# hila-chefer/Transformer-Explainability

Hardware: AMD Instinct MI355X
Metric: relevance maps/sec (ViT-B/16 224^2, batch 64 per GPU, generate_LRP transformer_attribution) (higher is better)
Workload: dtype f32 (3xbf16 split operands, 6 products, fp32 accumulate)

## Files before the change

include/te_relprop.h:

```cpp
#ifndef TE_RELPROP_H
#define TE_RELPROP_H

#include <stddef.h>
#include <stdint.h>

#ifdef __cplusplus
extern "C" {
#endif

typedef void* te_stream_t;
typedef uint16_t te_bf16_t;

enum {
  TE_OK = 0,
  TE_ERR_INVALID_ARG = -1,
  TE_ERR_WORKSPACE = -2,
  TE_ERR_UNSUPPORTED = -3,
  TE_ERR_NO_DEVICE = -4
};

enum { TE_VARIANT_OURS = 0, TE_VARIANT_LRP = 1, TE_IMPL_SIMPLE = 0x100 };

enum { TE_ROLLOUT_NORMALISE = 1, TE_ROLLOUT_CLS_FIXUP = 2, TE_ROLLOUT_ROW0 = 4 };

// ... 102 lines not shown
                                const float* R1, const float* s1, int64_t s1_stride,
                                const float* R2, const float* s2, int64_t s2_stride,
                                const float* X, float* out, int64_t B, int64_t n, te_stream_t stream);

int te_index_select_relprop_f32(const float* R, const float* X, float* out,
                                int64_t B, int64_t N, int64_t C, int64_t index, te_stream_t stream);

int te_gradcam_headmean_f32(const float* grad, const float* cam, float* out,
                            int64_t B, int64_t H, int64_t N, te_stream_t stream);

size_t te_rollout_workspace_bytes(int64_t L, int64_t B, int64_t N);
size_t te_rollout_row0_workspace_bytes(int64_t B, int64_t N);
int te_rollout_f32(const float* cams, int64_t L, int64_t start_layer, int64_t B, int64_t N,
                   int flags, float* joint, void* ws, size_t ws_bytes, te_stream_t stream);

#define TE_X6_TILE_AUTO 0
#define TE_X6_TILE_128 1
#define TE_X6_TILE_256 2
#define TE_X6_TILE_128x128 3
#define TE_X6_TEST_DROP_HANDOVER 0x200
#define TE_X6_WHOLE_TILES 0x10000
#define TE_X6_TEST_SMALL_GRID 0x4000
#define TE_X6_X_PLANES_SIGNED 0x20000
#define TE_X6_TILE_Z_SHIFT 10
#define TE_X6_TILE_C_SHIFT 12
#define TE_X6_PHASE_SPLIT 4
#define TE_X6_PHASE_Z 8
#define TE_X6_PHASE_C 16
#define TE_X6_PHASE_MASK 28
int te_linear_relprop_x6_supported(int64_t T, int64_t in_f, int64_t out_f);
size_t te_linear_relprop_x6_workspace_bytes(int64_t T, int64_t in_f, int64_t out_f);
size_t te_linear_x6_weight_planes_bytes(int64_t in_f, int64_t out_f);
size_t te_linear_x6_planes_bytes(int64_t rows, int64_t K);
int te_linear_x6_prepare_weights_f32(const float* W, int64_t in_f, int64_t out_f, void* planes, size_t planes_bytes,
                                     te_stream_t stream);
int te_linear_x6_split_abs_f32(const float* X, int64_t rows, int64_t K, void* planes, size_t planes_bytes,
                               te_stream_t stream);
int te_linear_relprop_x6_f32(const float* R, const float* r_scale, int64_t r_scale_stride, int64_t rows_per_sample,
                             const float* X, const float* W, const void* w_planes, const void* x_planes,
                             const float* Y, const float* bias, float* out,
                             int64_t T, int64_t in_f, int64_t out_f, int flags, unsigned* status, void* ws,
                             size_t ws_bytes, te_stream_t stream);
int te_linear_relprop_x6_check(const void* ws, int64_t T, int64_t in_f, int64_t out_f, te_stream_t stream);

int te_linear_relprop_x6_general_supported(int64_t T, int64_t in_f, int64_t out_f, int variant);
size_t te_linear_x6_weight_planes_lrp_bytes(int64_t in_f, int64_t out_f);
// ... 293 lines not shown
```

transformer-explainability_amd/csrc/te_api.hip:

```cpp
#include "te_common.h"

#include <string.h>

extern "C" int te_version(void) { return 706;  }

#ifndef TE_BUILD_ID
#define TE_BUILD_ID "unstamped"
#endif
extern "C" const char* te_build_id(void) { return TE_BUILD_ID; }

extern "C" const char* te_status_string(int status) {
  switch (status) {
    case TE_OK: return "ok";
    case TE_ERR_INVALID_ARG: return "invalid argument";
    case TE_ERR_WORKSPACE: return "workspace missing, misaligned or too small";
    case TE_ERR_UNSUPPORTED: return "shape not supported by the gfx950 kernels";
    case TE_ERR_NO_DEVICE: return "no gfx950 device visible";
    default: break;
  }
  if (status > 0) return hipGetErrorString((hipError_t)status);
  return "unknown status";
}

extern "C" int te_device_check(void) {
  int n = 0;
  if (hipGetDeviceCount(&n) != hipSuccess || n <= 0) return TE_ERR_NO_DEVICE;
  for (int d = 0; d < n; ++d) {
// ... 7 lines not shown
```

transformer-explainability_amd/csrc/te_linear_x6.hip:

```cpp
#include <algorithm>
#include <cmath>
#include <type_traits>

#include "te_x6.h"

namespace {

constexpr int kRB = 3 * kFrag;
constexpr int kMinFrag = 4;
constexpr float kCancelTol = 0.0078125f;
constexpr int kSpinMillis = 250;
constexpr int kErrWord = 1023;


enum { MODE_Z = 0, MODE_C = 1, MODE_G = 2, MODE_ZI = 3, MODE_Z1 = 4, MODE_CI = 5, MODE_X = 6, MODE_ZS = 7 };

__device__ __forceinline__ float bf16_f32(unsigned b) { return __uint_as_float(b << 16); }

enum { OP_ABS = 0, OP_POS = 1, OP_NEG = 2, OP_ID = 3 };
template <int OP>
__device__ __forceinline__ float apply_op(float x) {
  if constexpr (OP == OP_ID) return x;
  if constexpr (OP == OP_ABS) return __int_as_float(__float_as_int(x) & 0x7fffffff);
  const int b = __float_as_int(x);
  if constexpr (OP == OP_POS) return __int_as_float(b > 0 ? b : 0);
  return __int_as_float(b < 0 ? b : 0);
}

template <int OP, bool TRANSPOSE>
__global__ __launch_bounds__(256) void split_kernel(const float* __restrict__ src, unsigned char* __restrict__ dst,
                                                    int64_t R, int64_t K, int group, int sign,
                                                    unsigned char* __restrict__ dst_abs = nullptr) {
  const int r = threadIdx.x & 31, sl = threadIdx.x >> 5;
  const int64_t rb = blockIdx.x;
  const int64_t ks = (int64_t)blockIdx.y * 8 + sl;
  const int64_t nks = K >> 4;
  if (ks >= nks) return;
  const int64_t row = rb * 32 + r;
// ... 186 lines not shown
#else
#define X6_PASS4(a, b, c, d) (void)0
#endif

__device__ __forceinline__ void glds16(const unsigned char* src, unsigned char* lds_wave_base) {
  __builtin_amdgcn_global_load_lds((const __attribute__((address_space(1))) void*)src,
                                   (__attribute__((address_space(3))) void*)lds_wave_base, 16, 0, 0);
}

constexpr int kStages = 2;
template <int WM>
struct X6Geo {
  static constexpr int NWM = (WM == 1) ? 1 : 2, NWN = (WM == 0) ? 2 : 4, MI = (WM == 0) ? 2 : 4;
  static constexpr int NW = NWM * NWN, THREADS = 64 * NW, WPS = (WM == 0) ? 3 : 2;
  static constexpr int TM = NWM * MI * 32, TT = NWN * 64;
  static constexpr int NPA = 3 * NWM * MI, NPB = 3 * NWN * 2;
  static constexpr int ACC = MI * 2 * 16;
  static constexpr int MAX_SPX = (WM == 2) ? 32 : (WM == 1) ? 64 : 96;
};

template <int WM, int MODE>
struct X6Lds {
  using GEO = X6Geo<WM>;
  static constexpr bool STAGED = (MODE == MODE_Z || MODE == MODE_ZS || MODE == MODE_ZI || MODE == MODE_Z1) && GEO::MI == 4;
  static constexpr int STAGES = kStages * (GEO::NPA + GEO::NPB) * kFrag;
  static constexpr int MAIN = (STAGED && GEO::NW * 16384 > STAGES) ? GEO::NW * 16384 : STAGES;
  static constexpr int TOTAL = MAIN + GEO::NW * 512 + 16;
};

template <int WM, int MODE>
__global__ __launch_bounds__(X6Geo<WM>::THREADS, X6Geo<WM>::WPS) void x6_kernel(const X6Params p) {
  using GEO = X6Geo<WM>;
  constexpr int NW = GEO::NW, NWM = GEO::NWM, NWN = GEO::NWN, MI = GEO::MI;
  constexpr bool SGN = MODE == MODE_ZS;
  constexpr bool Z_ABS = MODE == MODE_Z || SGN;
  constexpr bool IS_Z = (Z_ABS || MODE == MODE_ZI || MODE == MODE_Z1);
  constexpr bool IS_C = (MODE == MODE_C || MODE == MODE_CI);
  constexpr int G = IS_C ? 6 : 3;
  constexpr int NPA = GEO::NPA, NPB = GEO::NPB;
  constexpr int NP = NPA + NPB;
  static_assert(NPA / 3 == NW, "each wave stages one weight-side block");
  constexpr int PBW = NPB / 3 / NW;
  constexpr int STAGE = NP * kFrag;
  constexpr int GROUPS = NPA / G;
  constexpr int LDS_MAIN = X6Lds<WM, MODE>::MAIN;
  extern __shared__ __attribute__((aligned(16))) unsigned char smem[];

  const int lane = threadIdx.x & 63;
  const int wave = __builtin_amdgcn_readfirstlane(threadIdx.x >> 6);
  const int wm = wave / NWN, wn = wave % NWN;
  const int lane16 = lane * 16;

  const int bid = blockIdx.x, spx = gridDim.x >> 3;
  const int xcd = bid & 7, slot = bid >> 3;
  const int nks = p.nks;
  const int tiles = p.ntm * p.ntn;
  const int tx0 = (int)((int64_t)tiles * xcd / 8), tx1 = (int)((int64_t)tiles * (xcd + 1) / 8);
  const int ntx = tx1 - tx0;
// ... 21 lines not shown
  for (int seq = 0; seq < nseq; ++seq) {
    int tile, k0, k1;
    if (head && seq == 0) {
      tile = l_tile, k0 = 0, k1 = ke;
    } else if (tail && seq == nseq - 1) {
      tile = f_tile, k0 = kb, k1 = (f_tile == l_tile) ? ke : nks;
    } else {
      tile = full0 + seq - (head ? 1 : 0), k0 = 0, k1 = nks;
    }
    tile += tx0;
    int tn, tm;
    if (p.t_fast) {
      tm = tile / p.ntn, tn = tile - tm * p.ntn;
    } else {
      tn = tile / p.ntm, tm = tile - tn * p.ntm;
    }

    const unsigned char* srcA;
    if constexpr (!IS_C)
      srcA = p.A + (int64_t)(tm * GROUPS + wave) * p.a_group_stride + (int64_t)k0 * kRB;
    else
      srcA = p.A + (int64_t)(tm * GROUPS + (wave >> 1)) * p.a_group_stride + (int64_t)k0 * (2 * kRB) + (wave & 1) * kRB;
    const unsigned char* srcB[PBW];
#pragma unroll
    for (int u = 0; u < PBW; ++u) {
      const int cb = min(tn * (GEO::TT / 32) + wave * PBW + u, p.ncb - 1);
      srcB[u] = p.B + (int64_t)cb * p.b_rb_stride + (int64_t)k0 * kRB;
    }
    unsigned char* const ldsA = smem + wave * kRB;
    unsigned char* const ldsB = smem + NPA * kFrag + wave * (PBW * kRB);
    u32x4 breg[SGN ? PBW : 1][3];
    auto stage_in = [&](int stg, int adv) __attribute__((always_inline)) {
      srcA += adv * (G * kFrag);
#pragma unroll
      for (int u = 0; u < PBW; ++u) srcB[u] += adv * kRB;
#pragma unroll
      for (int q = 0; q < 3; ++q) glds16(srcA + q * kFrag + lane16, ldsA + stg * STAGE + q * kFrag);
#pragma unroll
      for (int u = 0; u < PBW; ++u)
#pragma unroll
        for (int q = 0; q < 3; ++q) {
          if constexpr (SGN) breg[u][q] = *reinterpret_cast<const u32x4*>(srcB[u] + q * kFrag + lane16);
          else glds16(srcB[u] + q * kFrag + lane16, ldsB + stg * STAGE + (u * 3 + q) * kFrag);
        }
    };
    auto sign_and_store = [&](int stg) __attribute__((always_inline)) {
#pragma unroll
      for (int u = 0; u < (SGN ? PBW : 0); ++u) {
#pragma unroll
        for (int e = 0; e < 4; ++e) {
          const unsigned m = breg[u][0][e] & 0x80008000u;
          breg[u][0][e] &= 0x7fff7fffu;
          breg[u][1][e] ^= m;
          breg[u][2][e] ^= m;
        }
#pragma unroll
        for (int q = 0; q < 3; ++q) *reinterpret_cast<u32x4*>(ldsB + stg * STAGE + (u * 3 + q) * kFrag + lane16) = breg[u][q];
      }
    };

    auto wait_for = [&](unsigned* flag) -> bool {
      unsigned* const ok_word = reinterpret_cast<unsigned*>(smem + LDS_MAIN + NW * 512);
      if (threadIdx.x == 0) {
        unsigned spins = 0, ok = 1u;
        const long long t_begin = wall_clock64();
        while (__hip_atomic_load(flag, __ATOMIC_RELAXED, __HIP_MEMORY_SCOPE_AGENT) == 0u) {
          __builtin_amdgcn_s_sleep(8);
// ... 23 lines not shown
      for (int mi = 0; mi < MI; ++mi)
#pragma unroll
        for (int ni = 0; ni < 2; ++ni) {
#pragma unroll
          for (int c = 0; c < 4; ++c) {
            const f32x4 v = ip[c * 64];
#pragma unroll
            for (int e = 0; e < 4; ++e) acc[mi][ni][4 * c + e] = handed_over ? v[e] : __builtin_nanf("");
          }
          ip += 4 * 64;
          asm volatile("" : "+v"(ip));
        }
    } else {
#pragma unroll
      for (int mi = 0; mi < MI; ++mi)
#pragma unroll
        for (int ni = 0; ni < 2; ++ni)
#pragma unroll
          for (int e = 0; e < 16; ++e) acc[mi][ni][e] = 0.0f;
    }

    stage_in(0, 0);
    if constexpr (SGN) sign_and_store(0);
    int st = 0;
    bf16x8 a[MI][3], b[2][3];
    for (int ks = k0; ks < k1; ++ks) {
      asm volatile("s_waitcnt vmcnt(0) lgkmcnt(0)" ::: "memory");
      __builtin_amdgcn_s_barrier();
      const unsigned char* sA = smem + st * STAGE + wm * (MI * kRB) + lane16;
      const unsigned char* sB = smem + st * STAGE + NPA * kFrag + wn * (2 * kRB) + lane16;
      const unsigned aA = (unsigned)(uintptr_t)sA, aB = (unsigned)(uintptr_t)sB;
#define X6_SB __builtin_amdgcn_sched_barrier(0)
#define X6_RDB(ni, r) \
  asm volatile("ds_read_b128 %0, %1 offset:%2" : "=v"(b[ni][PB[r]]) : "v"(aB), "i"((ni) * kRB + PB[r] * kFrag))
#define X6_RDA(mi, r) \
  asm volatile("ds_read_b128 %0, %1 offset:%2" : "=v"(a[mi][PA[r]]) : "v"(aA), "i"((mi) * kRB + PA[r] * kFrag))
#define X6_WAIT(n)                                                           \
  X6_SB;                                                                     \
  asm volatile("s_waitcnt lgkmcnt(" #n ")" ::: "memory"); \
  X6_SB
#define X6_MM(mi, ni, q) acc[mi][ni] = TE_MFMA_BF16(a[mi][PA[q]], b[ni][PB[q]], acc[mi][ni])
#define X6_RD_HEAD(r) X6_SB; X6_RDB(0, r); X6_RDA(0, r); X6_RDA(1, r); X6_SB
#define X6_RD_TAIL(r) X6_SB; X6_RDB(1, r); X6_RDA(2, r); X6_RDA(3, r); X6_SB
      if constexpr (MI == 2) {
#define X6_RD4(r) X6_SB; X6_RDB(0, r); X6_RDA(0, r); X6_RDA(1, r); X6_RDB(1, r); X6_SB
        X6_RD4(0);
        X6_RD4(1);
        stage_in((st + 1) % kStages, (ks + 1 < k1) ? 1 : 0);
        X6_WAIT(6); X6_MM(0, 0, 0);
        X6_WAIT(5); X6_MM(1, 0, 0);
        X6_WAIT(4); X6_MM(1, 1, 0); X6_MM(0, 1, 0);
        X6_RD4(2);
        X6_WAIT(6); X6_MM(0, 0, 1);
        X6_WAIT(5); X6_MM(1, 0, 1);
        X6_WAIT(4); X6_MM(1, 1, 1); X6_MM(0, 1, 1);
        X6_WAIT(2); X6_MM(0, 0, 2);
        X6_WAIT(1); X6_MM(1, 0, 2);
        X6_WAIT(0); X6_MM(1, 1, 2); X6_MM(0, 1, 2);
        X6_SB;
#pragma unroll
        for (int q6 = 3; q6 < 6; ++q6) {
          X6_MM(0, 0, q6); X6_MM(1, 0, q6); X6_MM(1, 1, q6); X6_MM(0, 1, q6);
          X6_SB;
        }
#undef X6_RD4
      } else {
      X6_RD_HEAD(0);
      X6_RD_TAIL(0);
      stage_in((st + 1) % kStages, (ks + 1 < k1) ? 1 : 0);
      X6_WAIT(4); X6_MM(0, 0, 0);
      X6_WAIT(3); X6_MM(1, 0, 0);
      X6_WAIT(2); X6_MM(1, 1, 0); X6_MM(0, 1, 0);
      X6_RD_HEAD(1);
      X6_WAIT(4); X6_MM(2, 1, 0); X6_MM(2, 0, 0);
      X6_WAIT(3); X6_MM(3, 0, 0); X6_MM(3, 1, 0);
      X6_RD_TAIL(1);
      X6_WAIT(4); X6_MM(0, 0, 1);
      X6_WAIT(3); X6_MM(1, 0, 1);
      X6_WAIT(2); X6_MM(1, 1, 1); X6_MM(0, 1, 1);
      X6_RD_HEAD(2);
      X6_WAIT(4); X6_MM(2, 1, 1); X6_MM(2, 0, 1);
      X6_WAIT(3); X6_MM(3, 0, 1); X6_MM(3, 1, 1);
      X6_RD_TAIL(2);
      X6_WAIT(4); X6_MM(0, 0, 2);
      X6_WAIT(3); X6_MM(1, 0, 2);
      X6_WAIT(2); X6_MM(1, 1, 2); X6_MM(0, 1, 2);
      X6_WAIT(1); X6_MM(2, 1, 2); X6_MM(2, 0, 2);
      X6_WAIT(0); X6_MM(3, 0, 2); X6_MM(3, 1, 2);
      X6_SB;
#pragma unroll
      for (int q6 = 3; q6 < 6; ++q6) {
        X6_MM(0, 0, q6); X6_MM(1, 0, q6); X6_MM(1, 1, q6); X6_MM(0, 1, q6);
        X6_MM(2, 1, q6); X6_MM(2, 0, q6); X6_MM(3, 0, q6); X6_MM(3, 1, q6);
        X6_SB;
      }
      }
#undef X6_SB
#undef X6_RDB
#undef X6_RDA
#undef X6_WAIT
#undef X6_MM
#undef X6_RD_HEAD
#undef X6_RD_TAIL
      if constexpr (SGN) sign_and_store((st + 1) % kStages);
      st = (st + 1 == kStages) ? 0 : st + 1;
    }
    if constexpr (SGN) asm volatile("s_waitcnt lgkmcnt(0)" ::: "memory");

    auto publish = [&](float* dst, unsigned* flag) __attribute__((always_inline)) {
      f32x4* op = reinterpret_cast<f32x4*>(dst) + (size_t)wave * (GEO::ACC / 4) * 64 + lane;
#pragma unroll
      for (int mi = 0; mi < MI; ++mi)
#pragma unroll
        for (int ni = 0; ni < 2; ++ni) {
#pragma unroll
          for (int c = 0; c < 4; ++c) {
            f32x4 v;
#pragma unroll
            for (int e = 0; e < 4; ++e) v[e] = acc[mi][ni][4 * c + e];
            op[c * 64] = v;
          }
          op += 4 * 64;
          asm volatile("" : "+v"(op));
        }
      asm volatile("s_waitcnt vmcnt(0)" ::: "memory");
      __syncthreads();
      if (threadIdx.x == 0) {
        __builtin_amdgcn_fence(__ATOMIC_RELEASE, "agent");
        asm volatile("s_waitcnt vmcnt(0)" ::: "memory");
        if (!p.drop_handover) __hip_atomic_store(flag, 1u, __ATOMIC_RELAXED, __HIP_MEMORY_SCOPE_AGENT);
// ... 249 lines not shown
          if (__builtin_amdgcn_ballot_w64(bad != 0) != 0) {
            asm volatile("s_waitcnt vmcnt(0)" ::: "memory");
            const float* Rrow = p.R + tl[ni] * p.out_f;
#pragma clang loop unroll(disable)
            for (int e = 0; e < 16; ++e) {
              if ((bad >> e) & 1u) {
                const int jj = j0 + 8 * (e >> 2) + 4 * h + (e & 3);
                const float z = (MODE == MODE_ZI) ? exact_zi(p.X + tl[ni] * p.in_f, p.W + (int64_t)jj * p.in_f, p.in_f)
                                                  : exact_z(p.X + tl[ni] * p.in_f, p.W + (int64_t)jj * p.in_f, p.in_f);
                float rr = Rrow[jj];
                if (p.rs) rr = rr * f[ni];
                unsigned pl[3];
                split3(te_sd(rr, z), pl);
                unsigned short* d = reinterpret_cast<unsigned short*>(Srow + (int64_t)(jj >> 4) * kRB + ((jj >> 3) & 1) * 512) + (jj & 7);
                d[0] = (unsigned short)pl[0];
                d[kFrag / 2] = (unsigned short)pl[1];
                d[kFrag] = (unsigned short)pl[2];
              }
            }
          }
        }
      }
      }
    } else if constexpr (MODE == MODE_G) {
      float* const bias_lds = reinterpret_cast<float*>(smem + LDS_MAIN) + wave * 128;
      if (lane < MI * 8) {
        f32x4 bv = {0.0f, 0.0f, 0.0f, 0.0f};
        if (p.bias) bv = *reinterpret_cast<const f32x4*>(p.bias + (tm * (NWM * MI) + wm * MI) * 32 + lane * 4);
        *reinterpret_cast<f32x4*>(bias_lds + lane * 4) = bv;
      }
#pragma unroll
      for (int ni = 0; ni < 2; ++ni) {
        const int64_t t = ((int64_t)tn * (GEO::TT / 32) + wn * 2 + ni) * 32 + tc;
        float* orow = p.out + (t < p.T ? t : 0) * p.out_f + (tm * (NWM * MI) + wm * MI) * 32 + 4 * h;
#pragma unroll
        for (int mi = 0; mi < MI; ++mi)
#pragma unroll
          for (int g = 0; g < 4; ++g) {
            const f32x4 b4 = *reinterpret_cast<const f32x4*>(bias_lds + mi * 32 + 8 * g + 4 * h);
            f32x4 o;
#pragma unroll
            for (int c = 0; c < 4; ++c) o[c] = acc[mi][ni][4 * g + c] + b4[c];
            if (t < p.T) *reinterpret_cast<f32x4*>(orow + mi * 32 + 8 * g) = o;
          }
      }
    } else if constexpr (MODE == MODE_X) {
#pragma unroll
// ... 98 lines not shown
  l.s = xsets * l.x_stride;
  l.partial = l.s + ssets * l.s_stride;
  l.flags = l.partial + kPartialBytes;
  l.total = l.flags + passes * kFlagBytes;
  return l;
}
inline X6Workspace gemm_workspace(int64_t T, int64_t K, int64_t M) { return x6_workspace(T, K, M, 1, 0, 1); }
inline X6Workspace rule_workspace(int64_t T, int64_t in_f, int64_t out_f) { return x6_workspace(T, in_f, out_f, 1, 1, kRulePasses); }
inline X6Workspace general_workspace(int64_t T, int64_t in_f, int64_t out_f) { return x6_workspace(T, in_f, out_f, 2, 2, kGeneralPasses); }

struct X6WeightPlanes { size_t c, total; };
inline X6WeightPlanes weight_planes(int64_t in_f, int64_t out_f) {
  const size_t c = te_align_up(planes_bytes(out_f, in_f), 256);
  return {c, c + te_align_up(2 * planes_bytes(in_f, out_f), 256)};
}
struct X6WeightPlanesLrp { size_t wn, wpT, wnT, total; };
inline X6WeightPlanesLrp weight_planes_lrp(int64_t in_f, int64_t out_f) {
  const size_t za = te_align_up(planes_bytes(out_f, in_f), 256), ca = te_align_up(planes_bytes(in_f, out_f), 256);
  return {za, 2 * za, 2 * za + ca, 2 * za + 2 * ca};
}

constexpr int kTileMask = TE_X6_TILE_128 | TE_X6_TILE_256 | TE_X6_TILE_128x128;
constexpr int kProductFlags = kTileMask | TE_X6_WHOLE_TILES | TE_X6_TEST_DROP_HANDOVER | TE_X6_TEST_SMALL_GRID;
constexpr int kRuleFlags = kProductFlags | TE_X6_PHASE_MASK | TE_X6_X_PLANES_SIGNED | (kTileMask << TE_X6_TILE_Z_SHIFT) | (kTileMask << TE_X6_TILE_C_SHIFT);

inline int pick_wm(int64_t in_f, int64_t out_f) {
  if (out_f % 256 == 0 && in_f % 128 == 0) return 2;
  if (out_f % 128 == 0 && in_f % 64 == 0) return 1;
  return 0;
}

inline long long spin_ticks_for_current_device() {
  static long long cached[64] = {};
  int dev = 0;
  if (hipGetDevice(&dev) != hipSuccess || dev < 0 || dev >= 64) dev = 0;
  if (cached[dev] == 0) {
    int khz = 0;
    if (hipDeviceGetAttribute(&khz, hipDeviceAttributeWallClockRate, dev) != hipSuccess || khz <= 0) khz = 100000;
    cached[dev] = (long long)khz * kSpinMillis;
  }
  return cached[dev];
}

template <int WM, int MODE>
int launch_x6(const X6Params& p, hipStream_t stream) {
  using GEO = X6Geo<WM>;
  constexpr int lds = X6Lds<WM, MODE>::TOTAL;
// ... 167 lines not shown
  TE_RETURN_IF_LAUNCH_FAILED();
  return TE_OK;
}

extern "C" int te_gelu_forward_x6_planes_f32(const float* x, float* y, int64_t rows, int64_t K, void* planes, void* planes_abs,
                                             size_t planes_bytes_, te_stream_t stream_) {
  const int rc = check_producer(x && y && planes, te_aligned16(x) && te_aligned16(y),
                                te_aligned16(planes) && (!planes_abs || te_aligned16(planes_abs)), rows, K, planes_bytes_);
  if (rc != TE_OK) return rc;
  gelu_split_lds_kernel<SRC_GELU_FWD><<<producer_grid(rows, K), dim3(256), 0, (hipStream_t)stream_>>>(
      nullptr, x, y, (unsigned char*)planes, (unsigned char*)planes_abs, rows, K);
  TE_RETURN_IF_LAUNCH_FAILED();
  return TE_OK;
}

extern "C" size_t te_gemm_x6_workspace_bytes(int64_t T, int64_t K, int64_t M) {
  return te_gemm_x6_supported(T, K, M) ? gemm_workspace(T, K, M).total : 0;
}

extern "C" int te_gemm_x6_f32(const float* X, const void* x_planes, const void* w_planes, const float* bias, float* out,
                              int64_t T, int64_t K, int64_t M, int flags, unsigned* status, void* ws, size_t ws_bytes,
                              te_stream_t stream_) {
  if ((!X && !x_planes) || !w_planes || !out) return TE_ERR_INVALID_ARG;
  if ((flags & ~kProductFlags) != 0) return TE_ERR_INVALID_ARG;
  if (!te_gemm_x6_supported(T, K, M)) return TE_ERR_UNSUPPORTED;
  if (!ws || ws_bytes < te_gemm_x6_workspace_bytes(T, K, M) || !te_aligned16(ws)) return TE_ERR_WORKSPACE;
  if ((X && !te_aligned16(X)) || !te_aligned16(out) || !te_aligned16(w_planes) || (bias && !te_aligned16(bias)) ||
      (x_planes && !te_aligned16(x_planes)))
    return TE_ERR_UNSUPPORTED;
  hipStream_t stream = (hipStream_t)stream_;
  const X6Workspace l = gemm_workspace(T, K, M);
  zero_flag_regions(l.flag_region(ws, 0), 1, stream);
  if (!x_planes) {
    int rc = te_linear_x6_split_matrix_f32(X, T, K, 0, l.x(ws, 0), planes_bytes(T, K), stream_);
    if (rc != TE_OK) return rc;
    x_planes = l.x(ws, 0);
  }
  const int wm = choose_geo((M % 256 == 0) ? 2 : 1, T, M, flags & kTileMask, 192, true);
  const int rc = launch_pass<MODE_G>(call_params(T, l.acc(ws), bias, out, status, flags), wm, (const unsigned char*)w_planes,
                                     (const unsigned char*)x_planes, nullptr, K, M, l.flag_region(ws, 0), stream);
  if (rc != TE_OK) return rc;
  TE_RETURN_IF_LAUNCH_FAILED();
  return TE_OK;
}

extern "C" size_t te_linear_relprop_x6_workspace_bytes(int64_t T, int64_t in_f, int64_t out_f) {
  return te_linear_relprop_x6_supported(T, in_f, out_f) ? rule_workspace(T, in_f, out_f).total : 0;
}

extern "C" int te_linear_relprop_x6_f32(const float* R, const float* r_scale, int64_t r_scale_stride,
                                        int64_t rows_per_sample, const float* X, const float* W, const void* w_planes,
                                        const void* x_planes, const float* Y, const float* bias, float* out, int64_t T,
                                        int64_t in_f, int64_t out_f, int flags, unsigned* status, void* ws,
                                        size_t ws_bytes, te_stream_t stream_) {
  if (!R || !X || !W || !w_planes || !Y || !out || T <= 0) return TE_ERR_INVALID_ARG;
  if (!te_linear_relprop_x6_supported(T, in_f, out_f)) return TE_ERR_UNSUPPORTED;
  if (!ws || ws_bytes < te_linear_relprop_x6_workspace_bytes(T, in_f, out_f) || !te_aligned16(ws)) return TE_ERR_WORKSPACE;
  if (!te_aligned16(X) || !te_aligned16(W) || !te_aligned16(R) || !te_aligned16(Y) || !te_aligned16(out) ||
      !te_aligned16(w_planes) || (bias && !te_aligned16(bias)) || (x_planes && !te_aligned16(x_planes)))
    return TE_ERR_UNSUPPORTED;
  if (bad_r_scale(r_scale, rows_per_sample, T)) return TE_ERR_INVALID_ARG;
  if ((flags & ~kRuleFlags) != 0) return TE_ERR_INVALID_ARG;
  const int phases = (flags & TE_X6_PHASE_MASK) ? (flags & TE_X6_PHASE_MASK) : TE_X6_PHASE_MASK;
  hipStream_t stream = (hipStream_t)stream_;
  const X6Workspace l = rule_workspace(T, in_f, out_f);
  unsigned char* Ss = l.sp(ws, 0);
  const unsigned char* wz = (const unsigned char*)w_planes;
  const unsigned char* wc = wz + weight_planes(in_f, out_f).c;

  if (phases & TE_X6_PHASE_SPLIT) zero_flag_regions(l.flag_region(ws, 0), kRulePasses, stream);
  const bool x_signed = (flags & TE_X6_X_PLANES_SIGNED) != 0;
  if (!x_planes) {
    if (phases & TE_X6_PHASE_SPLIT) {
      int rc = x_signed ? te_linear_x6_split_matrix_f32(X, T, in_f, 0, l.x(ws, 0), planes_bytes(T, in_f), stream_)
                        : te_linear_x6_split_abs_f32(X, T, in_f, l.x(ws, 0), planes_bytes(T, in_f), stream_);
      if (rc != TE_OK) return rc;
    }
    x_planes = l.x(ws, 0);
  }
  const int wm_max = pick_wm(in_f, out_f);
  const int pz = (flags >> TE_X6_TILE_Z_SHIFT) & kTileMask, pc = (flags >> TE_X6_TILE_C_SHIFT) & kTileMask;
  const int wm_z = choose_geo(wm_max, T, out_f, pz ? pz : (flags & kTileMask), 256, true);
  const int wm_c = choose_geo(wm_max, T, 2 * in_f, pc ? pc : (flags & kTileMask));
  const X6Params p = rule_params(call_params(T, l.acc(ws), bias, out, status, flags), R, r_scale, r_scale_stride, rows_per_sample,
                                 X, W, Y);
  int rc;
  if (phases & TE_X6_PHASE_Z) {
    rc = x_signed ? launch_pass<MODE_ZS>(p, wm_z, wz, (const unsigned char*)x_planes, Ss, in_f, out_f, l.flag_region(ws, 0), stream, 1.0f)
                  : launch_pass<MODE_Z>(p, wm_z, wz, (const unsigned char*)x_planes, Ss, in_f, out_f, l.flag_region(ws, 0), stream, 1.0f);
    if (rc != TE_OK) return rc;
  }
  if (phases & TE_X6_PHASE_C) {
    rc = launch_pass<MODE_C>(p, wm_c, wc, Ss, Ss, in_f, out_f, l.flag_region(ws, 1), stream, 1.0f);
    if (rc != TE_OK) return rc;
  }
  TE_RETURN_IF_LAUNCH_FAILED();
  return TE_OK;
}

extern "C" int te_linear_relprop_x6_general_supported(int64_t T, int64_t in_f, int64_t out_f, int variant) {
  if (!te_linear_relprop_x6_supported(T, in_f, out_f)) return 0;
  if (variant == TE_VARIANT_LRP) return (in_f % 128 == 0) ? 1 : 0;
  return variant == TE_VARIANT_OURS ? 1 : 0;
}

extern "C" size_t te_linear_x6_weight_planes_lrp_bytes(int64_t in_f, int64_t out_f) {
  return te_linear_relprop_x6_general_supported(1, in_f, out_f, TE_VARIANT_LRP) ? weight_planes_lrp(in_f, out_f).total : 0;
}

extern "C" int te_linear_x6_prepare_weights_lrp_f32(const float* W, int64_t in_f, int64_t out_f, void* planes,
                                                    size_t planes_bytes_, te_stream_t stream_) {
// ... 116 lines not shown
```

transformer-explainability_amd/ops.py:

```python
from __future__ import annotations

import contextlib
import os
from typing import Optional, Sequence, Tuple

import torch

from . import _lib
from ._lib import (TE_HEADMEAN_CLAMP, TE_HEADMEAN_ROW0, TE_IMPL_SIMPLE, TE_RATIONALE_CLAMP, TE_ROLLOUT_CLS_FIXUP,
                   TE_ROLLOUT_NORMALISE, TE_ROLLOUT_ROW0, TE_VARIANT_LRP, TE_VARIANT_OURS)
from ._lib import (TE_X6_PHASE_C, TE_X6_PHASE_SPLIT, TE_X6_PHASE_Z, TE_X6_TEST_DROP_HANDOVER,
                   TE_X6_TEST_SMALL_GRID, TE_X6_TILE_C_SHIFT, TE_X6_TILE_Z_SHIFT, TE_X6_WHOLE_TILES, TE_X6_X_PLANES_SIGNED)

Tensor = torch.Tensor
_VARIANTS = {"ours": TE_VARIANT_OURS, "lrp": TE_VARIANT_LRP}

FORCE_SIMPLE = False
KERNEL_TIMER = None
_NULL = contextlib.nullcontext()


def _timed(name: str, flops: float = 0.0, nbytes: float = 0.0):
    return _NULL if KERNEL_TIMER is None else KERNEL_TIMER(name, float(flops), float(nbytes))


class Deferred:
    __slots__ = ("t", "scale")

    def __init__(self, t: Tensor, scale: Tensor):
        self.t, self.scale = t, scale

    @property
    def shape(self):
        return self.t.shape

# ... 227 lines not shown
    with _on_device(Wc) as lib:
        planes = _ws(getattr(lib, bytes_fn)(*dims), Wc)
        _lib.check(getattr(lib, prepare_fn)(_ptr(Wc), *dims, *extra, _ptr(planes), planes.numel(), _stream(Wc)), prepare_fn)
    return planes


def x6_weight_planes(W: Tensor, cache: Optional[dict] = None) -> Tensor:
    out_f, in_f = W.shape
    return _cached_planes(W, cache, "x6_planes", lambda Wd: (_prepare_planes(
        _c(Wd), "te_linear_x6_weight_planes_bytes", "te_linear_x6_prepare_weights_f32", (in_f, out_f)),))[0]


X6_GEMM = {"": "all", "1": "all", "0": "off"}.get(os.environ.get("TE_X6_GEMM", "all"), os.environ.get("TE_X6_GEMM", "all"))
if X6_GEMM not in ("all", "auto", "off"):
    raise ValueError(f"TE_X6_GEMM={X6_GEMM!r}: expected all / auto / off (or 1 / 0)")


def gemm_x6_wanted(T: int, K: int, M: int) -> bool:
    if X6_GEMM == "off" or T < 256 or not gemm_x6_supported(T, K, M):
        return False
    return X6_GEMM == "all" or (K <= 1024 and M >= 2 * K)


def x6_weight_planes_lrp(W: Tensor, cache: Optional[dict] = None) -> Tensor:
    out_f, in_f = W.shape
    return _cached_planes(W, cache, "x6_planes_lrp", lambda Wd: (_prepare_planes(
        _c(Wd), "te_linear_x6_weight_planes_lrp_bytes", "te_linear_x6_prepare_weights_lrp_f32", (in_f, out_f)),))[0]


def x6_matrix_planes(W: Tensor, transposed: bool, cache: Optional[dict] = None) -> Tensor:
    out_f, in_f = W.shape
    dims = (in_f, out_f) if transposed else (out_f, in_f)
    return _cached_planes(W, cache, "x6_gemm_planes_T" if transposed else "x6_gemm_planes", lambda Wd: (_prepare_planes(
        _c(Wd), "te_linear_x6_planes_bytes", "te_linear_x6_split_matrix_f32", dims, int(transposed)),))[0]


def linear_relprop_x6_supported(T: int, in_f: int, out_f: int) -> bool:
    return bool(_lib.load().te_linear_relprop_x6_supported(int(T), int(in_f), int(out_f)))


def gemm_x6_supported(T: int, K: int, M: int) -> bool:
    return bool(_lib.load().te_gemm_x6_supported(int(T), int(K), int(M)))


X6_KEEP_ABS = os.environ.get("TE_X6_KEEP_ABS", "1") not in ("", "0")
X6_SIGNED_PLANES = True
# ... 71 lines not shown
    hit = cache.pop("dy_planes_from_consumer", None)
    if hit is not None and dy.data_ptr() == hit[0].data_ptr() and tuple(dy.shape) == hit[1] and not any(dy.stride()):
        return hit[2]
    return None


def rule_takes_abs_planes(T: int, in_f: int, out_f: int) -> bool:
    return bool(USE_LINEAR_X6 and X6_KEEP_ABS and linear_relprop_x6_supported(T, in_f, out_f))


def gemm_x6(X: Tensor, w_planes: Tensor, bias: Optional[Tensor], M: int, timer_name: str = "gemm_x6",
            keep_abs: Optional[dict] = None, x_planes: Optional[Tensor] = None) -> Tensor:
    K = X.shape[-1]
    lead = X.shape[:-1]
    T = X.numel() // K
    Xc = None if x_planes is not None else _c(X).reshape(-1, K)
    like = X if Xc is None else Xc
    out = torch.empty((T, M), dtype=torch.float32, device=X.device)
    bc = None if bias is None else _c(bias.detach())
    with _on_device(like) as lib:
        ws = _ws(lib.te_gemm_x6_workspace_bytes(T, K, M), like)
        x_bytes = (6.0 if x_planes is not None else 10.0) * T * K
        xs = x_planes
        if xs is None and keep_abs is not None:
            got = take_x_planes(keep_abs, X, T, K)
            if got is not None:
                xs, x_bytes = got[0], 6.0 * T * K
                post_x_abs_planes(keep_abs, X, T, K, got[1] if got[1] is not None else _signed(xs))
        if xs is not None and xs.numel() * xs.element_size() < lib.te_linear_x6_planes_bytes(T, K):
            raise _lib.TeError(f"gemm_x6: the operand planes handed in hold {xs.numel() * xs.element_size()} bytes, "
                               f"[{T}, {K}] needs {lib.te_linear_x6_planes_bytes(T, K)}")
        for_rule = xs is None and keep_abs is not None and rule_takes_abs_planes(T, K, M)
        if for_rule and not X6_SIGNED_PLANES:
            x_bytes += 6.0 * T * K
        with _timed(timer_name, 12.0 * T * K * M, x_bytes + 6.0 * K * M + 4.0 * T * M):
            if for_rule:
                nb = lib.te_linear_x6_planes_bytes(T, K)
                if X6_SIGNED_PLANES:
                    xs = _signed(_ws(nb, Xc))
                    _lib.check(lib.te_linear_x6_split_matrix_f32(_ptr(Xc), T, K, 0, _ptr(xs), nb, _stream(Xc)),
                               "te_linear_x6_split_matrix_f32")
                    post_x_abs_planes(keep_abs, X, T, K, xs)
                else:
                    xs, xa = _ws(nb, Xc), _ws(nb, Xc)
                    _lib.check(lib.te_linear_x6_split_dual_f32(_ptr(Xc), T, K, _ptr(xs), _ptr(xa), nb, _stream(Xc)),
                               "te_linear_x6_split_dual_f32")
                    post_x_abs_planes(keep_abs, X, T, K, xa)
            _lib.check(lib.te_gemm_x6_f32(_ptr(Xc) if Xc is not None else None, _ptr(xs), _ptr(w_planes), _ptr(bc), _ptr(out),
                                          T, K, M, (X6_TILE | X6_FLAGS) & ~0x3c00, _ptr(x6_status(X.device)), _ptr(ws),
                                          ws.numel(), _stream(like)), "te_gemm_x6_f32")
    return out.reshape(*lead, M)


def linear_relprop(R: Tensor, X: Tensor, W: Tensor, alpha: float = 1.0, variant="ours",
                   Y: Optional[Tensor] = None, bias: Optional[Tensor] = None, cache: Optional[dict] = None) -> Tensor:
    if _any_f64(R, X, W):
        return linear_relprop_f64(R, X, W, alpha=alpha, variant=variant)
    if _is_bf16(X) or _is_bf16(W):
        return linear_relprop_bf16(R, X, W, alpha=alpha, variant=variant, cache=cache)
    out_f, in_f = W.shape
    lead = X.shape[:-1]
    R, r_scale = _split_deferred(R)
    Rc, Xc, Wc = _c(R).reshape(-1, out_f), _c(X).reshape(-1, in_f), _c(W)
    T = Xc.shape[0]
    if Rc.shape[0] != T:
        raise _lib.TeError(f"Linear.relprop: R has {Rc.shape[0]} rows, X has {T}")
    out = torch.empty((T, in_f), dtype=torch.float32, device=X.device)
    var = _variant(variant)
    fast_ok = (var == TE_VARIANT_OURS and alpha == 1 and in_f % 4 == 0 and out_f % 4 == 0 and
               all(t.data_ptr() % 16 == 0 for t in (Rc, Xc, Wc)))
    fwd = fast_ok and USE_FORWARD_OUTPUT and Y is not None
    if r_scale is not None and not fwd:
# ... 22 lines not shown
        gemm = 2.0 * T * in_f * out_f
        halves = 2 if alpha != 1 else 1
        units = (18.0 if var_code == TE_VARIANT_OURS else 24.0) * halves
        with _on_device(Xc) as lib, _timed("linear_x6_general", units * gemm,
                                           halves * (6.0 * (2 * T * in_f + 3 * in_f * out_f + 2 * T * out_f) + 16.0 * T * in_f)):
            ws = _ws(lib.te_linear_relprop_x6_general_workspace_bytes(T, in_f, out_f, var_code), Xc)
            _lib.check(lib.te_linear_relprop_x6_general_f32(_ptr(Rc), rs_ptr, rs_stride, rps, _ptr(Xc), _ptr(Wc), _ptr(wp),
                                                            _ptr(wpl), _ptr(xa), _ptr(Yg), _ptr(bg), _ptr(out), T, in_f,
                                                            out_f, float(alpha), var_code, (X6_TILE | X6_FLAGS) & ~0x3c00,
                                                            _ptr(x6_status(Xc.device)), _ptr(ws), ws.numel(), _stream(Xc)),
                       "te_linear_relprop_x6_general_f32")
            if X6_CHECK:
                x6_raise_if_failed(Xc.device)
        return out.reshape(*lead, in_f)
    if fwd:
        Yc = _c(Y.detach()).reshape(-1, out_f)
        bc = None if bias is None else _c(bias.detach())
        if Yc.shape[0] != T:
            raise _lib.TeError(f"Linear.relprop: Y has {Yc.shape[0]} rows, X has {T}")
    if (fwd and USE_LINEAR_X6 and Yc.data_ptr() % 16 == 0 and (bc is None or bc.data_ptr() % 16 == 0)
            and _lib.load().te_linear_relprop_x6_supported(T, in_f, out_f)):
        planes = x6_weight_planes(W, cache)
        xa = take_x_abs_planes(cache, X, T, in_f) if cache is not None else None
        x_signed = TE_X6_X_PLANES_SIGNED if planes_are_signed(xa) else 0
        with _on_device(Xc) as lib:
            ws = _ws(lib.te_linear_relprop_x6_workspace_bytes(T, in_f, out_f), Xc)
            status = x6_status(Xc.device)

            def call(flags):
                _lib.check(lib.te_linear_relprop_x6_f32(_ptr(Rc), rs_ptr, rs_stride, rps, _ptr(Xc), _ptr(Wc), _ptr(planes),
                                                        _ptr(xa), _ptr(Yc), _ptr(bc), _ptr(out), T, in_f, out_f,
                                                        X6_TILE | X6_FLAGS | x_signed | flags, _ptr(status), _ptr(ws), ws.numel(),
                                                        _stream(Xc)),
                           "te_linear_relprop_x6_f32")
            if KERNEL_TIMER is None:
                call(0)
            else:
                gemm = 2.0 * T * in_f * out_f
                if xa is None:
                    with _timed("linear_x6_split", 0.0, 10.0 * T * in_f):
                        call(TE_X6_PHASE_SPLIT)
                else:
                    call(TE_X6_PHASE_SPLIT)
                with _timed("linear_x6_zpass", 6.0 * gemm, 6.0 * (T * in_f + in_f * out_f + T * out_f) + 8.0 * T * out_f):
                    call(TE_X6_PHASE_Z)
                with _timed("linear_x6_cpass", 12.0 * gemm, 6.0 * (T * out_f + 2 * in_f * out_f) + 8.0 * T * in_f):
                    call(TE_X6_PHASE_C)
            if X6_CHECK:
                rc = lib.te_linear_relprop_x6_check(_ptr(ws), T, in_f, out_f, _stream(Xc))
                if rc != 0:
                    status.zero_()
                    raise _lib.TeError(f"te_linear_relprop_x6_f32({T},{in_f},{out_f}): a workgroup waited in vain for the "
                                       f"accumulators of a shared tile (status {rc}); the result is invalid")
                x6_raise_if_failed(Xc.device)
        return out.reshape(*lead, in_f)
    if KERNEL_TIMER is not None and fast_ok:
        with _on_device(Xc) as lib:
            S = torch.empty((T, out_f), dtype=torch.float32, device=X.device)
            st = _stream(Xc)
            if fwd:
                with _timed("linear_zpass_fwd", 2.0 * T * in_f * out_f, 4.0 * (T * in_f + 3 * T * out_f + in_f * out_f)):
                    _lib.check(lib.te_linear_zpass_fwd_scaled_f32(_ptr(Rc), rs_ptr, rs_stride, rps, _ptr(Xc), _ptr(Wc),
                                                                  _ptr(Yc), _ptr(bc), _ptr(S), T, in_f, out_f, st),
                               "te_linear_zpass_fwd_scaled_f32")
            else:
                with _timed("linear_zpass", 2.0 * T * (2 * in_f) * out_f, 4.0 * (T * in_f + 2 * T * out_f + in_f * out_f)):
                    _lib.check(lib.te_linear_zpass_f32(_ptr(Rc), _ptr(Xc), _ptr(Wc), _ptr(S), T, in_f, out_f, st),
# ... 1707 lines not shown
```

Before: 1044.

## Split activations into bf16 planes inside the x6 GEMM and Z-pass kernels

Measured after the change: 1051 (median of 6 runs). No clear change (+0.7%).

```diff
diff --git a/include/te_relprop.h b/include/te_relprop.h
--- a/include/te_relprop.h
+++ b/include/te_relprop.h
@@ -148,6 +148,7 @@
 #define TE_X6_WHOLE_TILES 0x10000
 #define TE_X6_TEST_SMALL_GRID 0x4000
 #define TE_X6_X_PLANES_SIGNED 0x20000
+#define TE_X6_X_DIRECT 0x80000
 #define TE_X6_TILE_Z_SHIFT 10
 #define TE_X6_TILE_C_SHIFT 12
 #define TE_X6_PHASE_SPLIT 4
diff --git a/transformer-explainability_amd/csrc/te_api.hip b/transformer-explainability_amd/csrc/te_api.hip
--- a/transformer-explainability_amd/csrc/te_api.hip
+++ b/transformer-explainability_amd/csrc/te_api.hip
@@ -2,7 +2,7 @@
 
 #include <string.h>
 
-extern "C" int te_version(void) { return 706;  }
+extern "C" int te_version(void) { return 707;  }
 
 #ifndef TE_BUILD_ID
 #define TE_BUILD_ID "unstamped"
diff --git a/transformer-explainability_amd/csrc/te_linear_x6.hip b/transformer-explainability_amd/csrc/te_linear_x6.hip
--- a/transformer-explainability_amd/csrc/te_linear_x6.hip
+++ b/transformer-explainability_amd/csrc/te_linear_x6.hip
@@ -13,7 +13,7 @@
 constexpr int kErrWord = 1023;
 
 
-enum { MODE_Z = 0, MODE_C = 1, MODE_G = 2, MODE_ZI = 3, MODE_Z1 = 4, MODE_CI = 5, MODE_X = 6, MODE_ZS = 7 };
+enum { MODE_Z = 0, MODE_C = 1, MODE_G = 2, MODE_ZI = 3, MODE_Z1 = 4, MODE_CI = 5, MODE_X = 6, MODE_ZS = 7, MODE_GD = 8, MODE_ZD = 9 };
 
 __device__ __forceinline__ float bf16_f32(unsigned b) { return __uint_as_float(b << 16); }
 
@@ -246,7 +246,7 @@
 template <int WM, int MODE>
 struct X6Lds {
   using GEO = X6Geo<WM>;
-  static constexpr bool STAGED = (MODE == MODE_Z || MODE == MODE_ZS || MODE == MODE_ZI || MODE == MODE_Z1) && GEO::MI == 4;
+  static constexpr bool STAGED = (MODE == MODE_Z || MODE == MODE_ZS || MODE == MODE_ZD || MODE == MODE_ZI || MODE == MODE_Z1) && GEO::MI == 4;
   static constexpr int STAGES = kStages * (GEO::NPA + GEO::NPB) * kFrag;
   static constexpr int MAIN = (STAGED && GEO::NW * 16384 > STAGES) ? GEO::NW * 16384 : STAGES;
   static constexpr int TOTAL = MAIN + GEO::NW * 512 + 16;
@@ -257,7 +257,9 @@
   using GEO = X6Geo<WM>;
   constexpr int NW = GEO::NW, NWM = GEO::NWM, NWN = GEO::NWN, MI = GEO::MI;
   constexpr bool SGN = MODE == MODE_ZS;
-  constexpr bool Z_ABS = MODE == MODE_Z || SGN;
+  constexpr bool DIR = MODE == MODE_GD || MODE == MODE_ZD;
+  constexpr bool Z_ABS = MODE == MODE_Z || SGN || MODE == MODE_ZD;
+  constexpr bool IS_G = MODE == MODE_G || MODE == MODE_GD;
   constexpr bool IS_Z = (Z_ABS || MODE == MODE_ZI || MODE == MODE_Z1);
   constexpr bool IS_C = (MODE == MODE_C || MODE == MODE_CI);
   constexpr int G = IS_C ? 6 : 3;
@@ -325,27 +327,91 @@
     else
       srcA = p.A + (int64_t)(tm * GROUPS + (wave >> 1)) * p.a_group_stride + (int64_t)k0 * (2 * kRB) + (wave & 1) * kRB;
     const unsigned char* srcB[PBW];
+    const unsigned char* srcX[DIR ? PBW : 1];
+    bool xlive[DIR ? PBW : 1];
+    unsigned xlane[DIR ? PBW : 1];
+    unsigned alane = lane16;
+#if defined(__HIP_DEVICE_COMPILE__)
+    if constexpr (DIR) asm volatile("" : "+v"(alane));
+#endif
 #pragma unroll
     for (int u = 0; u < PBW; ++u) {
-      const int cb = min(tn * (GEO::TT / 32) + wave * PBW + u, p.ncb - 1);
-      srcB[u] = p.B + (int64_t)cb * p.b_rb_stride + (int64_t)k0 * kRB;
+      if constexpr (DIR) {
+        const int cb = tn * (GEO::TT / 32) + wave * PBW + u;
+        const int64_t row0 = (int64_t)min(cb, p.ncb - 1) * 32;
+        xlive[u] = (int64_t)cb * 32 + (lane & 31) < p.T;
+        const int64_t row = min(row0 + (lane & 31), p.T - 1);
+        xlane[u] = ((unsigned)(row - row0) * (unsigned)nks * 16u + (unsigned)(lane >> 5) * 8u) * 4u;
+#if defined(__HIP_DEVICE_COMPILE__)
+        asm volatile("" : "+v"(xlane[u]));
+#endif
+        srcX[u] = reinterpret_cast<const unsigned char*>(p.X + row0 * ((int64_t)nks * 16) + (int64_t)k0 * 16);
+      } else {
+        const int cb = min(tn * (GEO::TT / 32) + wave * PBW + u, p.ncb - 1);
+        srcB[u] = p.B + (int64_t)cb * p.b_rb_stride + (int64_t)k0 * kRB;
+      }
     }
     unsigned char* const ldsA = smem + wave * kRB;
     unsigned char* const ldsB = smem + NPA * kFrag + wave * (PBW * kRB);
+    constexpr int kSplitRounds = 2;
     u32x4 breg[SGN ? PBW : 1][3];
+    f32x4 xreg[DIR ? PBW : 1][2];
     auto stage_in = [&](int stg, int adv) __attribute__((always_inline)) {
       srcA += adv * (G * kFrag);
 #pragma unroll
-      for (int u = 0; u < PBW; ++u) srcB[u] += adv * kRB;
-#pragma unroll
-      for (int q = 0; q < 3; ++q) glds16(srcA + q * kFrag + lane16, ldsA + stg * STAGE + q * kFrag);
-#pragma unroll
-      for (int u = 0; u < PBW; ++u)
-#pragma unroll
-        for (int q = 0; q < 3; ++q) {
-          if constexpr (SGN) breg[u][q] = *reinterpret_cast<const u32x4*>(srcB[u] + q * kFrag + lane16);
-          else glds16(srcB[u] + q * kFrag + lane16, ldsB + stg * STAGE + (u * 3 + q) * kFrag);
-        }
+      for (int u = 0; u < PBW; ++u) {
+        if constexpr (DIR) srcX[u] += adv * 64;
+        else srcB[u] += adv * kRB;
+      }
+#pragma unroll
+      for (int q = 0; q < 3; ++q) glds16(srcA + q * kFrag + (DIR ? alane : (unsigned)lane16), ldsA + stg * STAGE + q * kFrag);
+#pragma unroll
+      for (int u = 0; u < PBW; ++u) {
+        if constexpr (DIR) {
+          xreg[u][0] = *reinterpret_cast<const f32x4*>(srcX[u] + xlane[u]);
+          xreg[u][1] = *reinterpret_cast<const f32x4*>(srcX[u] + xlane[u] + 16);
+        } else {
+#pragma unroll
+          for (int q = 0; q < 3; ++q) {
+            if constexpr (SGN) breg[u][q] = *reinterpret_cast<const u32x4*>(srcB[u] + q * kFrag + lane16);
+            else glds16(srcB[u] + q * kFrag + lane16, ldsB + stg * STAGE + (u * 3 + q) * kFrag);
+          }
+        }
+      }
+    };
+    u32x4 xpl[DIR ? PBW : 1][3];
+    auto split_and_store = [&](int stg, int part) __attribute__((always_inline)) {
+      constexpr int NPAIR = DIR ? PBW * 4 : 0;
+#pragma unroll
+      for (int i = NPAIR * part / kSplitRounds; i < NPAIR * (part + 1) / kSplitRounds; ++i) {
+        const int u = i >> 2, e = i & 3;
+        unsigned pk[3];
+        float x0 = xreg[u][e >> 1][2 * (e & 1)], x1 = xreg[u][e >> 1][2 * (e & 1) + 1];
+#if defined(__HIP_DEVICE_COMPILE__)
+        asm volatile("" : "+v"(x0), "+v"(x1));
+#endif
+        x0 = xlive[u] ? x0 : 0.0f;
+        x1 = xlive[u] ? x1 : 0.0f;
+        if constexpr (MODE == MODE_ZD) split3_pk(apply_op<OP_ABS>(x0), apply_op<OP_ABS>(x1), pk);
+        else split3_pk(x0, x1, pk);
+#pragma unroll
+        for (int q = 0; q < 3; ++q) xpl[u][q][e] = pk[q];
+      }
+      if (part == kSplitRounds - 1) {
+#pragma unroll
+        for (int u = 0; u < (DIR ? PBW : 0); ++u)
+#pragma unroll
+          for (int q = 0; q < 3; ++q) *reinterpret_cast<u32x4*>(ldsB + stg * STAGE + (u * 3 + q) * kFrag + lane16) = xpl[u][q];
+      }
+    };
+    auto split_round = [&](int stg, int part) __attribute__((always_inline)) {
+      split_and_store(stg, part);
+      constexpr int NMF = MI * 2, PER = (PBW * 4 + kSplitRounds - 1) / kSplitRounds * 13;
+#pragma unroll
+      for (int i = 0; i < NMF; ++i) {
+        __builtin_amdgcn_sched_group_barrier(0x008, 1, 0);
+        __builtin_amdgcn_sched_group_barrier(0x002, (PER + NMF - 1) / NMF, 0);
+      }
     };
     auto sign_and_store = [&](int stg) __attribute__((always_inline)) {
 #pragma unroll
@@ -415,6 +481,10 @@
 
     stage_in(0, 0);
     if constexpr (SGN) sign_and_store(0);
+    if constexpr (DIR) {
+#pragma unroll
+      for (int part = 0; part < kSplitRounds; ++part) split_and_store(0, part);
+    }
     int st = 0;
     bf16x8 a[MI][3], b[2][3];
     for (int ks = k0; ks < k1; ++ks) {
@@ -454,6 +524,7 @@
 #pragma unroll
         for (int q6 = 3; q6 < 6; ++q6) {
           X6_MM(0, 0, q6); X6_MM(1, 0, q6); X6_MM(1, 1, q6); X6_MM(0, 1, q6);
+          if constexpr (DIR) if (q6 >= 6 - kSplitRounds) split_round((st + 1) % kStages, q6 - (6 - kSplitRounds));
           X6_SB;
         }
 #undef X6_RD4
@@ -485,6 +556,7 @@
       for (int q6 = 3; q6 < 6; ++q6) {
         X6_MM(0, 0, q6); X6_MM(1, 0, q6); X6_MM(1, 1, q6); X6_MM(0, 1, q6);
         X6_MM(2, 1, q6); X6_MM(2, 0, q6); X6_MM(3, 0, q6); X6_MM(3, 1, q6);
+        if constexpr (DIR) if (q6 >= 6 - kSplitRounds) split_round((st + 1) % kStages, q6 - (6 - kSplitRounds));
         X6_SB;
       }
       }
@@ -498,7 +570,7 @@
       if constexpr (SGN) sign_and_store((st + 1) % kStages);
       st = (st + 1 == kStages) ? 0 : st + 1;
     }
-    if constexpr (SGN) asm volatile("s_waitcnt lgkmcnt(0)" ::: "memory");
+    if constexpr (SGN || DIR) asm volatile("s_waitcnt lgkmcnt(0)" ::: "memory");
 
     auto publish = [&](float* dst, unsigned* flag) __attribute__((always_inline)) {
       f32x4* op = reinterpret_cast<f32x4*>(dst) + (size_t)wave * (GEO::ACC / 4) * 64 + lane;
@@ -794,7 +866,7 @@
         }
       }
       }
-    } else if constexpr (MODE == MODE_G) {
+    } else if constexpr (IS_G) {
       float* const bias_lds = reinterpret_cast<float*>(smem + LDS_MAIN) + wave * 128;
       if (lane < MI * 8) {
         f32x4 bv = {0.0f, 0.0f, 0.0f, 0.0f};
@@ -939,7 +1011,8 @@
 
 constexpr int kTileMask = TE_X6_TILE_128 | TE_X6_TILE_256 | TE_X6_TILE_128x128;
 constexpr int kProductFlags = kTileMask | TE_X6_WHOLE_TILES | TE_X6_TEST_DROP_HANDOVER | TE_X6_TEST_SMALL_GRID;
-constexpr int kRuleFlags = kProductFlags | TE_X6_PHASE_MASK | TE_X6_X_PLANES_SIGNED | (kTileMask << TE_X6_TILE_Z_SHIFT) | (kTileMask << TE_X6_TILE_C_SHIFT);
+constexpr int kGemmFlags = kProductFlags | TE_X6_X_DIRECT;
+constexpr int kRuleFlags = kGemmFlags | TE_X6_PHASE_MASK | TE_X6_X_PLANES_SIGNED | (kTileMask << TE_X6_TILE_Z_SHIFT) | (kTileMask << TE_X6_TILE_C_SHIFT);
 
 inline int pick_wm(int64_t in_f, int64_t out_f) {
   if (out_f % 256 == 0 && in_f % 128 == 0) return 2;
@@ -1153,7 +1226,9 @@
                               int64_t T, int64_t K, int64_t M, int flags, unsigned* status, void* ws, size_t ws_bytes,
                               te_stream_t stream_) {
   if ((!X && !x_planes) || !w_planes || !out) return TE_ERR_INVALID_ARG;
-  if ((flags & ~kProductFlags) != 0) return TE_ERR_INVALID_ARG;
+  if ((flags & ~kGemmFlags) != 0) return TE_ERR_INVALID_ARG;
+  const bool direct = (flags & TE_X6_X_DIRECT) != 0;
+  if (direct && (x_planes || !X)) return TE_ERR_INVALID_ARG;
   if (!te_gemm_x6_supported(T, K, M)) return TE_ERR_UNSUPPORTED;
   if (!ws || ws_bytes < te_gemm_x6_workspace_bytes(T, K, M) || !te_aligned16(ws)) return TE_ERR_WORKSPACE;
   if ((X && !te_aligned16(X)) || !te_aligned16(out) || !te_aligned16(w_planes) || (bias && !te_aligned16(bias)) ||
@@ -1162,14 +1237,17 @@
   hipStream_t stream = (hipStream_t)stream_;
   const X6Workspace l = gemm_workspace(T, K, M);
   zero_flag_regions(l.flag_region(ws, 0), 1, stream);
-  if (!x_planes) {
+  if (!x_planes && !direct) {
     int rc = te_linear_x6_split_matrix_f32(X, T, K, 0, l.x(ws, 0), planes_bytes(T, K), stream_);
     if (rc != TE_OK) return rc;
     x_planes = l.x(ws, 0);
   }
   const int wm = choose_geo((M % 256 == 0) ? 2 : 1, T, M, flags & kTileMask, 192, true);
-  const int rc = launch_pass<MODE_G>(call_params(T, l.acc(ws), bias, out, status, flags), wm, (const unsigned char*)w_planes,
-                                     (const unsigned char*)x_planes, nullptr, K, M, l.flag_region(ws, 0), stream);
+  X6Params p = call_params(T, l.acc(ws), bias, out, status, flags);
+  p.X = X;
+  const int rc = direct ? launch_pass<MODE_GD>(p, wm, (const unsigned char*)w_planes, nullptr, nullptr, K, M, l.flag_region(ws, 0), stream)
+                        : launch_pass<MODE_G>(p, wm, (const unsigned char*)w_planes, (const unsigned char*)x_planes, nullptr, K, M,
+                                              l.flag_region(ws, 0), stream);
   if (rc != TE_OK) return rc;
   TE_RETURN_IF_LAUNCH_FAILED();
   return TE_OK;
@@ -1192,6 +1270,8 @@
     return TE_ERR_UNSUPPORTED;
   if (bad_r_scale(r_scale, rows_per_sample, T)) return TE_ERR_INVALID_ARG;
   if ((flags & ~kRuleFlags) != 0) return TE_ERR_INVALID_ARG;
+  const bool direct = (flags & TE_X6_X_DIRECT) != 0;
+  if (direct && (x_planes || (flags & TE_X6_X_PLANES_SIGNED))) return TE_ERR_INVALID_ARG;
   const int phases = (flags & TE_X6_PHASE_MASK) ? (flags & TE_X6_PHASE_MASK) : TE_X6_PHASE_MASK;
   hipStream_t stream = (hipStream_t)stream_;
   const X6Workspace l = rule_workspace(T, in_f, out_f);
@@ -1201,7 +1281,7 @@
 
   if (phases & TE_X6_PHASE_SPLIT) zero_flag_regions(l.flag_region(ws, 0), kRulePasses, stream);
   const bool x_signed = (flags & TE_X6_X_PLANES_SIGNED) != 0;
-  if (!x_planes) {
+  if (!x_planes && !direct) {
     if (phases & TE_X6_PHASE_SPLIT) {
       int rc = x_signed ? te_linear_x6_split_matrix_f32(X, T, in_f, 0, l.x(ws, 0), planes_bytes(T, in_f), stream_)
                         : te_linear_x6_split_abs_f32(X, T, in_f, l.x(ws, 0), planes_bytes(T, in_f), stream_);
@@ -1217,7 +1297,8 @@
                                  X, W, Y);
   int rc;
   if (phases & TE_X6_PHASE_Z) {
-    rc = x_signed ? launch_pass<MODE_ZS>(p, wm_z, wz, (const unsigned char*)x_planes, Ss, in_f, out_f, l.flag_region(ws, 0), stream, 1.0f)
+    rc = direct   ? launch_pass<MODE_ZD>(p, wm_z, wz, nullptr, Ss, in_f, out_f, l.flag_region(ws, 0), stream, 1.0f)
+         : x_signed ? launch_pass<MODE_ZS>(p, wm_z, wz, (const unsigned char*)x_planes, Ss, in_f, out_f, l.flag_region(ws, 0), stream, 1.0f)
                   : launch_pass<MODE_Z>(p, wm_z, wz, (const unsigned char*)x_planes, Ss, in_f, out_f, l.flag_region(ws, 0), stream, 1.0f);
     if (rc != TE_OK) return rc;
   }
diff --git a/transformer-explainability_amd/ops.py b/transformer-explainability_amd/ops.py
--- a/transformer-explainability_amd/ops.py
+++ b/transformer-explainability_amd/ops.py
@@ -10,7 +10,8 @@
 from ._lib import (TE_HEADMEAN_CLAMP, TE_HEADMEAN_ROW0, TE_IMPL_SIMPLE, TE_RATIONALE_CLAMP, TE_ROLLOUT_CLS_FIXUP,
                    TE_ROLLOUT_NORMALISE, TE_ROLLOUT_ROW0, TE_VARIANT_LRP, TE_VARIANT_OURS)
 from ._lib import (TE_X6_PHASE_C, TE_X6_PHASE_SPLIT, TE_X6_PHASE_Z, TE_X6_TEST_DROP_HANDOVER,
-                   TE_X6_TEST_SMALL_GRID, TE_X6_TILE_C_SHIFT, TE_X6_TILE_Z_SHIFT, TE_X6_WHOLE_TILES, TE_X6_X_PLANES_SIGNED)
+                   TE_X6_TEST_SMALL_GRID, TE_X6_TILE_C_SHIFT, TE_X6_TILE_Z_SHIFT, TE_X6_WHOLE_TILES, TE_X6_X_DIRECT,
+                   TE_X6_X_PLANES_SIGNED)
 
 Tensor = torch.Tensor
 _VARIANTS = {"ours": TE_VARIANT_OURS, "lrp": TE_VARIANT_LRP}
@@ -284,6 +285,21 @@
     return X6_GEMM == "all" or (K <= 1024 and M >= 2 * K)
 
 
+X6_DIRECT_X = True
+
+
+def x6_direct_wanted(T: int, K: int, M: int, which: str) -> bool:
+    if which not in ("product", "zpass"):
+        raise ValueError(f"x6_direct_wanted: which = {which!r}")
+    if which == "product" and T < X6_DIRECT_MIN_ROWS:
+        return False
+    return bool(X6_DIRECT_X) and (which, K, M) not in X6_DIRECT_EXCEPT
+
+
+X6_DIRECT_EXCEPT: frozenset = frozenset({("product", 768, 3072), ("zpass", 768, 3072)})
+X6_DIRECT_MIN_ROWS = 12608
+
+
 def x6_weight_planes_lrp(W: Tensor, cache: Optional[dict] = None) -> Tensor:
     out_f, in_f = W.shape
     return _cached_planes(W, cache, "x6_planes_lrp", lambda Wd: (_prepare_planes(
@@ -401,6 +417,7 @@
         ws = _ws(lib.te_gemm_x6_workspace_bytes(T, K, M), like)
         x_bytes = (6.0 if x_planes is not None else 10.0) * T * K
         xs = x_planes
+        stray = keep_abs is not None and "x_planes_from_producer" in keep_abs
         if xs is None and keep_abs is not None:
             got = take_x_planes(keep_abs, X, T, K)
             if got is not None:
@@ -410,6 +427,10 @@
             raise _lib.TeError(f"gemm_x6: the operand planes handed in hold {xs.numel() * xs.element_size()} bytes, "
                                f"[{T}, {K}] needs {lib.te_linear_x6_planes_bytes(T, K)}")
         for_rule = xs is None and keep_abs is not None and rule_takes_abs_planes(T, K, M)
+        direct = (xs is None and not stray and x6_direct_wanted(T, K, M, "product")
+                  and (not for_rule or x6_direct_wanted(T, K, M, "zpass")))
+        if direct:
+            for_rule, x_bytes = False, 4.0 * T * K
         if for_rule and not X6_SIGNED_PLANES:
             x_bytes += 6.0 * T * K
         with _timed(timer_name, 12.0 * T * K * M, x_bytes + 6.0 * K * M + 4.0 * T * M):
@@ -426,7 +447,8 @@
                                "te_linear_x6_split_dual_f32")
                     post_x_abs_planes(keep_abs, X, T, K, xa)
             _lib.check(lib.te_gemm_x6_f32(_ptr(Xc) if Xc is not None else None, _ptr(xs), _ptr(w_planes), _ptr(bc), _ptr(out),
-                                          T, K, M, (X6_TILE | X6_FLAGS) & ~0x3c00, _ptr(x6_status(X.device)), _ptr(ws),
+                                          T, K, M, (X6_TILE | X6_FLAGS) & ~0x3c00 | (TE_X6_X_DIRECT if direct else 0),
+                                          _ptr(x6_status(X.device)), _ptr(ws),
                                           ws.numel(), _stream(like)), "te_gemm_x6_f32")
     return out.reshape(*lead, M)
 
@@ -495,7 +517,9 @@
             and _lib.load().te_linear_relprop_x6_supported(T, in_f, out_f)):
         planes = x6_weight_planes(W, cache)
         xa = take_x_abs_planes(cache, X, T, in_f) if cache is not None else None
-        x_signed = TE_X6_X_PLANES_SIGNED if planes_are_signed(xa) else 0
+        x_src = TE_X6_X_PLANES_SIGNED if planes_are_signed(xa) else 0
+        if xa is None and x6_direct_wanted(T, in_f, out_f, "zpass"):
+            x_src = TE_X6_X_DIRECT
         with _on_device(Xc) as lib:
             ws = _ws(lib.te_linear_relprop_x6_workspace_bytes(T, in_f, out_f), Xc)
             status = x6_status(Xc.device)
@@ -503,19 +527,21 @@
             def call(flags):
                 _lib.check(lib.te_linear_relprop_x6_f32(_ptr(Rc), rs_ptr, rs_stride, rps, _ptr(Xc), _ptr(Wc), _ptr(planes),
                                                         _ptr(xa), _ptr(Yc), _ptr(bc), _ptr(out), T, in_f, out_f,
-                                                        X6_TILE | X6_FLAGS | x_signed | flags, _ptr(status), _ptr(ws), ws.numel(),
+                                                        X6_TILE | X6_FLAGS | x_src | flags, _ptr(status), _ptr(ws), ws.numel(),
                                                         _stream(Xc)),
                            "te_linear_relprop_x6_f32")
             if KERNEL_TIMER is None:
                 call(0)
             else:
                 gemm = 2.0 * T * in_f * out_f
-                if xa is None:
+                direct = x_src == TE_X6_X_DIRECT
+                if xa is None and not direct:
                     with _timed("linear_x6_split", 0.0, 10.0 * T * in_f):
                         call(TE_X6_PHASE_SPLIT)
                 else:
                     call(TE_X6_PHASE_SPLIT)
-                with _timed("linear_x6_zpass", 6.0 * gemm, 6.0 * (T * in_f + in_f * out_f + T * out_f) + 8.0 * T * out_f):
+                with _timed("linear_x6_zpass", 6.0 * gemm,
+                            (4.0 if direct else 6.0) * T * in_f + 6.0 * (in_f * out_f + T * out_f) + 8.0 * T * out_f):
                     call(TE_X6_PHASE_Z)
                 with _timed("linear_x6_cpass", 12.0 * gemm, 6.0 * (T * out_f + 2 * in_f * out_f) + 8.0 * T * in_f):
                     call(TE_X6_PHASE_C)
```
